# rajan-dubey8/camouflage-multimodal

Hardware: AMD Instinct MI355X
Metric: images/sec fwd+bwd (fusion model train step: fwd + loss + bwd + clip + AdamW) (higher is better)
Workload: dtype bf16; 1 GPU; BASELINE configs[1] on the path that exists (SURVEY 8d): cross-attention fusion model, packed variable-Nr minibatch (Nr ~ real 303..530 histogram, mean 483), Nk=13 real KG rows, train mode dropout 0.3, random-init weights; batch_per_gpu=16, global_batch=16, rg_dim=128, hidden_dim=256, num_heads=8, parallelism=dp1, precision=bf16 MFMA operands, fp32 accumulate/optimizer

## Files before the change

### camouflage_multimodal_amd/csrc/fused_rows.hip

```cpp
#include "fused_rows.h"
#include "shadow_inl.h"
#include "gemm.h"
#include "mfma_inl.h"

namespace {

template <int NT, int KS, bool W_IS_A, int DEPTH, bool USE_ROT = true>
struct Stage {
  static constexpr int TOTAL = NT * KS;
  static constexpr int D = DEPTH < TOTAL ? DEPTH : TOTAL;
  static_assert(!USE_ROT || (KS & (KS - 1)) == 0, "rotated k order: power-of-two k steps");
  u32x4 buf[D];
  const u32x4* wp; int rot;
  __device__ __forceinline__ int keff(int ks) const { return USE_ROT ? ((ks + rot) & (KS - 1)) : ks; }
  __device__ __forceinline__ const u32x4* wptr(int i) const { return wp + 64 * (keff(i / NT) * NT + (i % NT)); }
  __device__ __forceinline__ void prefetch(const u32x4* __restrict__ wp_, int rot_) {
    wp = wp_; rot = rot_;
#pragma unroll
    for (int i = 0; i < D; ++i) buf[i] = *wptr(i);
  }
  __device__ __forceinline__ void run(const char* act, f32x16 (&acc)[NT]) {
    run_f([&](int ks) { return *reinterpret_cast<const bf16x8*>(act + 32 * ks); }, acc);
  }
  template <class F>
// ... 967 lines not shown

constexpr int SLAB_TILES = 10;

template <int DEPTH, bool ROT>
__global__ __launch_bounds__(256, 2) void bwd2_kernel(const Bwd2Args a) {
  extern __shared__ __attribute__((aligned(16))) char smem[];
  const int tid = threadIdx.x, lane = tid & 63, l31 = lane & 31, h = lane >> 5;
  const int w = __builtin_amdgcn_readfirstlane(tid >> 6);
  const int Nk = a.Nk;
  char* Q2s = smem + X_Q2S; char* dO2s = smem + X_DO2S; float* tabs = reinterpret_cast<float*>(smem + X_TABS);
  char* bufT = smem + X_BUFT; char* imgs = smem + X_IMGS;
  int* flag = reinterpret_cast<int*>(smem + X_RED);
  const int xb = (int)blockIdx.x - a.B - a.rg_tiles_max, xearly = (a.kg_split - 1) * a.B;
  if (xb >= xearly) { ln_slab_sum(a, xb - xearly); return; }
  stamp(a.stamps, 0);
  const bool early = (int)blockIdx.x < a.B || xb >= 0;
  int b;
  if (early) {
    b = xb >= 0 ? xb % a.B : (int)blockIdx.x;
    const int kq = xb >= 0 ? 1 + xb / a.B : 0;
    const int r_lo = a.kg_split > 1 ? min(4 * kq, Nk) : 0, r_hi = a.kg_split > 1 ? min(4 * kq + 4, Nk) : Nk;
    const size_t krow0 = (size_t)b * Nk;
    Stage<2, 32, true, DEPTH, false> se;
    se.prefetch(reinterpret_cast<const u32x4*>(a.WcKgT) + (size_t)w * (48 * 2 * 64) + 64 * (16 * 2) + lane, 0);
    u32x2 du2reg[2][4];
#pragma unroll
    for (int t = 0; t < 2; ++t)
#pragma unroll
      for (int g = 0; g < 4; ++g) du2reg[t][g] = *reinterpret_cast<const u32x2*>(a.dU2_16 + (krow0 + min(l31, Nk - 1)) * 256 + 64 * w + 32 * t + 8 * g + 4 * h);
    const int t0 = a.tile_off[b], t1 = a.tile_off[b + 1];
    for (int c = tid; c < 32 * 64; c += 256) {
      const int j = c >> 6, ch = c & 63;
      u32x4 v = u32x4{0u, 0u, 0u, 0u};
      if (j >= r_lo && j < r_hi) {
        float4 x0, x1;
        if (a.slabs & 2) {
          x0 = x1 = make_float4(0.f, 0.f, 0.f, 0.f);
          const float* src = a.slabKV + (size_t)j * 512 + 8 * ch;
          for (int tb = t0; tb < t1; tb += SLAB_TILES) {
            float4 p0[SLAB_TILES], p1[SLAB_TILES];
#pragma unroll
            for (int u = 0; u < SLAB_TILES; ++u) {
              const float* s = src + (size_t)min(tb + u, t1 - 1) * Nk * 512;
              p0[u] = *reinterpret_cast<const float4*>(s); p1[u] = *reinterpret_cast<const float4*>(s + 4);
            }
#pragma unroll
            for (int u = 0; u < SLAB_TILES; ++u) {
              const bool ok = tb + u < t1;
              x0.x += ok ? p0[u].x : 0.f; x0.y += ok ? p0[u].y : 0.f; x0.z += ok ? p0[u].z : 0.f; x0.w += ok ? p0[u].w : 0.f;
              x1.x += ok ? p1[u].x : 0.f; x1.y += ok ? p1[u].y : 0.f; x1.z += ok ? p1[u].z : 0.f; x1.w += ok ? p1[u].w : 0.f;
            }
          }
          float* dst = a.dKV + (krow0 + j) * 512 + 8 * ch;
          *reinterpret_cast<float4*>(dst) = x0; *reinterpret_cast<float4*>(dst + 4) = x1;
        } else {
          const float* src = a.dKV + (krow0 + j) * 512 + 8 * ch;
          x0 = *reinterpret_cast<const float4*>(src); x1 = *reinterpret_cast<const float4*>(src + 4);
        }
        v = u32x4{pack2(x0.x, x0.y), pack2(x0.z, x0.w), pack2(x1.x, x1.y), pack2(x1.z, x1.w)};
      }
      *reinterpret_cast<u32x4*>(bufT + j * PQ + 512 + 16 * ch) = v;
    }
    __syncthreads();
    f32x16 acc[2] = {zero16(), zero16()};
    se.run(bufT + l31 * PQ + 512 + 16 * h, acc);
    copy_out<6>(bufT + r_lo * PQ, PQ, 512, a.dQKVkg16 + 256, 768, krow0 + r_lo, r_hi - r_lo);
    if (a.kg_defer) {
      us16* const dGp16 = reinterpret_cast<us16*>(a.dGpart);
      if (l31 >= r_lo && l31 < r_hi) {
#pragma unroll
        for (int t = 0; t < 2; ++t)
#pragma unroll
          for (int g = 0; g < 4; ++g) {
            const int c0 = 64 * w + 32 * t + 8 * g + 4 * h;
            const u32x2 uv = du2reg[t][g];
            *reinterpret_cast<u32x2*>(dGp16 + (krow0 + l31) * 256 + c0) =
                u32x2{pack2(acc[t][4 * g] + bf_lo(uv.x), acc[t][4 * g + 1] + bf_hi(uv.x)), pack2(acc[t][4 * g + 2] + bf_lo(uv.y), acc[t][4 * g + 3] + bf_hi(uv.y))};
          }
      }
      if (b == a.B - 1 && kq == 0) {
        const size_t tk = (size_t)a.B * Nk, n16 = (((tk + 127) & ~size_t(127)) - tk) * 32;
        for (size_t c = tid; c < n16; c += 256) *(reinterpret_cast<u32x4*>(dGp16 + tk * 256) + c) = u32x4{0u, 0u, 0u, 0u};
      }
    } else if (l31 >= r_lo && l31 < r_hi) {
#pragma unroll
      for (int t = 0; t < 2; ++t)
#pragma unroll
        for (int g = 0; g < 4; ++g) {
          const int c0 = 64 * w + 32 * t + 8 * g + 4 * h;
          const u32x2 uv = du2reg[t][g];
          float* dst = a.dGpart + (krow0 + l31) * 256 + c0;
          __hip_atomic_store(dst, acc[t][4 * g] + bf_lo(uv.x), __ATOMIC_RELAXED, __HIP_MEMORY_SCOPE_AGENT);
          __hip_atomic_store(dst + 1, acc[t][4 * g + 1] + bf_hi(uv.x), __ATOMIC_RELAXED, __HIP_MEMORY_SCOPE_AGENT);
          __hip_atomic_store(dst + 2, acc[t][4 * g + 2] + bf_lo(uv.y), __ATOMIC_RELAXED, __HIP_MEMORY_SCOPE_AGENT);
          __hip_atomic_store(dst + 3, acc[t][4 * g + 3] + bf_hi(uv.y), __ATOMIC_RELAXED, __HIP_MEMORY_SCOPE_AGENT);
        }
    }
  } else {
  const int4 td = a.tile_desc[(int)blockIdx.x - a.B];
  if (td.x < 0) return;
  b = td.x;
  const size_t rowg0 = td.y;
  const int nrows = td.z;
  const bool rok = l31 < nrows;
  const size_t vrow = rowg0 + min(l31, nrows - 1);
  Stage<2, 48, true, DEPTH, false> sr;
  sr.prefetch(reinterpret_cast<const u32x4*>(a.WcRgT) + (size_t)w * (48 * 2 * 64) + lane, 0);
// ... 451 lines not shown
  Bwd1Args k = a;
  if (kg_only) { k.rg_tiles_max = 0; k.stamps = nullptr; }
  const dim3 grid(k.B + k.rg_tiles_max + k.writer_blocks + k.nzero + k.twg.tiles);
  const double rows = (kg_only ? 0.0 : (double)a.rows_rg) + (double)a.B * a.Nk;
  const int prof = gemm_prof_open(stream, 2.0 * rows * (512.0 * 256.0 + 256.0 * 256.0) + (kg_only ? 0.0 : 10.0 * (double)a.rows_rg * a.Nk * 256.0), PROF_BWD1);
  if (variant == 0) launch_lds<bwd1_kernel<12, false>>(grid, dim3(256), W_LDS, stream, k);
  else              launch_lds<bwd1_kernel<12, true>>(grid, dim3(256), W_LDS, stream, k);
  gemm_prof_close(prof, stream);
  return (int)hipGetLastError();
}

size_t fused_bwd2_lds() { return X_LDS; }

int launch_fused_bwd2(Bwd2Args& a, int variant, hipStream_t stream) {
  (void)variant;
  if (a.B < 1 || a.Nk < 1 || a.Nk > 16 || a.rg_tiles_max < 1 || !a.Q2_16 || !a.dO2_16 || !a.lse2 || !a.delta2 || !a.KV2_16 || !a.dQKV16 ||
      !a.dU16 || !a.WcRgT || !a.dR16 || !a.dQ2acc || !a.dKV || !a.dU2_16 || !a.WcKgT || !a.dQKVkg16 || !a.dG16 || !a.dGpart || !a.tickets || !a.off || !a.tile_off || !a.tile_desc)
    return (int)hipErrorInvalidValue;
  if (!al16(a.dQKV16) || !al16(a.dQKVkg16) || !al16(a.WcRgT) || !al16(a.WcKgT) || !al16(a.dQ2acc) || !al16(a.dKV)) return (int)hipErrorInvalidValue;
  if (a.slabs && (a.param_space || (a.slabs & ~3) || !a.slabKV || !a.slabLN || !a.ln_dgamma[0] || !a.ln_dgamma[1] || !a.ln_dbeta[0] || !a.ln_dbeta[1]))
    return (int)hipErrorInvalidValue;
  if (a.param_space) a.kg_defer = 0;
  else if (a.kg_defer < 0) a.kg_defer = a.B * a.Nk <= FUSED_BWD2_DEFER_MAX_TK ? 1 : 0;
  const double dr = 2.0 * ((double)a.rows_rg * 768.0 + (double)a.B * a.Nk * (a.kg_defer ? 512.0 : 768.0)) * 256.0;
  const int prof = gemm_prof_open(stream, (a.param_space ? 0.0 : dr) + 10.0 * (double)a.rows_rg * a.Nk * 256.0, PROF_BWD2);
  if (!a.param_space) a.split_finish = 0;
  a.kg_split = (a.slabs & 2) ? 4 : 1;
  if (!a.param_space) launch_lds<bwd2_kernel<12, false>>(dim3(a.kg_split * a.B + a.rg_tiles_max + ((a.slabs & 1) ? 4 : 0)), dim3(256), X_LDS, stream, a);
  else                launch_lds<bwd2p_kernel<12, false>>(dim3(a.B + a.rg_tiles_max), dim3(256), X_LDS, stream, a);
  if (a.split_finish) hipLaunchKernelGGL(bwd2_finish_kernel, dim3(a.B), dim3(256), 0, stream, a);
  gemm_prof_close(prof, stream);
  return (int)hipGetLastError();
}
```

### camouflage_multimodal_amd/csrc/fusion_abi.hip

```cpp
#include <hip/hip_runtime.h>

#include <algorithm>
#include <cmath>
#include <cstdio>
#include <cstring>
#include <string>

#include "../../include/camo_fusion.h"

#include "attn.h"
#include "gemm.h"
#include "fused_rows.h"
#include "tail_wide.h"
#include "attn_maps.h"
#include "gemm16.h"
#include "misc.h"
#include "abi_util.h"
#include "fusion_ws.h"

namespace {
thread_local std::string g_err;
}

int camo_abi::fail(int code, const std::string& msg) { g_err = msg; return code; }
// ... 627 lines not shown
  }
  if (pl.bwd1 == CAMO_BWD1_64) CK(launch_wide2_bwd1(a1, x.opt->fused_variant, st), "fused backward, first half (64-row half-blocks)");
  else                         CK(launch_fused_bwd1(a1, x.opt->fused_variant, st), "fused backward, first half");
  if (pl.tail_event == CAMO_EVENT_AFTER_BWD1) CK(record_tail_event(c, st), "tail event");
  Bwd2Args a2; std::memset(&a2, 0, sizeof(a2));
  a2.Q2_16 = f.Q2_16; a2.dO2_16 = f.dO2_16; a2.lse2 = f.lse2; a2.delta2 = f.delta2; a2.KV2_16 = f.KV2_16; a2.dQKV16 = f.dQKV16;
  a2.dU16 = f.dU16; a2.WcRgT = sh.WcRgT; a2.dR16 = f.dR16; a2.dQ2acc = w.dQ2acc; a2.dKV = w.dKV;
  a2.slabs = a1.slabs; a2.slabKV = f.slabKV; a2.slabLN = f.slabLN;
  for (int i = 0; i < 2; ++i) { a2.ln_dgamma[i] = a1.s[i].dgamma; a2.ln_dbeta[i] = a1.s[i].dbeta; }
  a2.dU2_16 = f.dU2_16; a2.WcKgT = sh.WcKgT; a2.dQKVkg16 = f.dQKVkg16; a2.dG16 = f.dG16; a2.dGpart = f.dGpart;
  a2.tickets = w.tickets + B; a2.off = rg_offsets; a2.tile_off = bd.tile_off; a2.tile_desc = bd.tile_desc;
  a2.B = B; a2.Nk = Nk; a2.rows_rg = T; a2.rg_tiles_max = T / 32 + B; a2.qscale = a1.qscale; a2.drop = drop;
  a2.stamps = g_dbg_stamps ? g_dbg_stamps + (size_t)3 * g_dbg_stamp_blocks * 8 : nullptr;
  const bool param_space = pl.param_space != 0;
  a2.param_space = param_space ? 1 : 0;
  a2.split_finish = pl.bwd2 != CAMO_BWD2_ROWS32 ? 1 : 0;
  a2.kg_defer = x.opt->exp == 32 ? 0 : (x.opt->exp == 64 ? 1 : (x.opt->tn_big > 0 ? 0 : -1));
  if (pl.bwd2 == CAMO_BWD2_64) CK(launch_wide2_bwd2(a2, st), "fused backward, second half (64-row blocks)");
  else CK(launch_fused_bwd2(a2, x.opt->fused_variant, st), "fused backward, second half");
  if (!param_space) {
    GB16 g(drop, *x.opt, st);
    const bool kgq = a2.kg_defer == 1;
    if (kgq) {
      Gemm16Prob& p = g.tn(nullptr, H, f.KG16, D, Gr[CAMO_P_KG_PROJ_W], D, Gr[CAMO_P_KG_PROJ_B], H, D, TK);
      p.A = reinterpret_cast<const us*>(w.dQ2acc); p.flags |= GF_A_F32 | GF_KGQ;
      p.kgq_wT = sh.WcKgT; p.kgq_w = P[CAMO_P_A2_IN_W]; p.ldg = H;
      p.C16 = f.dG16; p.ldc16 = H; p.kgq_part16 = reinterpret_cast<const us*>(f.dGpart); p.kgq_a16 = f.dQKVkg16; p.kgq_lda16 = 3 * H;
    }
    g.tn(f.dH16, 2 * H, f.Y16, H, Gr[CAMO_P_F1_W0], H, Gr[CAMO_P_F1_B0], 2 * H, H, T);
    g.tn(f.dU16, H, f.O16, H, Gr[CAMO_P_A1_OUT_W], H, Gr[CAMO_P_A1_OUT_B], H, H, T);
    g.tn(f.dQKV16, 3 * H, f.R16, H, Gr[CAMO_P_A1_IN_W], H, Gr[CAMO_P_A1_IN_B], H, H, T);
    g.tn(f.dQKV16 + H, 3 * H, f.R16, H, Gr[CAMO_P_A2_IN_W] + HH, H, Gr[CAMO_P_A2_IN_B] + H, 2 * H, H, T);
    g.tn(f.dR16, H, f.X16, D, Gr[CAMO_P_RG_PROJ_W], D, Gr[CAMO_P_RG_PROJ_B], H, D, T);
    g.tn(f.dH2_16, 2 * H, f.Y2_16, H, Gr[CAMO_P_F2_W0], H, Gr[CAMO_P_F2_B0], 2 * H, H, TK);
    g.tn(f.dU2_16, H, f.O2_16, H, Gr[CAMO_P_A2_OUT_W], H, Gr[CAMO_P_A2_OUT_B], H, H, TK);
    if (kgq) {
      Gemm16Prob& p = g.tn(nullptr, H, f.G16, H, Gr[CAMO_P_A2_IN_W], H, Gr[CAMO_P_A2_IN_B], H, H, TK);
      p.A = reinterpret_cast<const us*>(w.dQ2acc); p.flags |= GF_A_F32;
    } else {
      g.tn(f.dQKVkg16, 3 * H, f.G16, H, Gr[CAMO_P_A2_IN_W], H, Gr[CAMO_P_A2_IN_B], H, H, TK);
    }
    g.tn(f.dQKVkg16 + H, 3 * H, f.G16, H, Gr[CAMO_P_A1_IN_W] + HH, H, Gr[CAMO_P_A1_IN_B] + H, 2 * H, H, TK);
    g.tn(kgq ? reinterpret_cast<const us*>(f.dGpart) : f.dG16, H, f.KG16, D, Gr[CAMO_P_KG_PROJ_W], D, Gr[CAMO_P_KG_PROJ_B], H, D, TK);
    CK(g.run(), "node-level weight gradients");
    return 0;
  }
  float* const Mrg = w.parM.Mrg; float* const Mkg = w.parM.Mkg; float* const dbrg = w.parM.dbrg; float* const dbkg = w.parM.dbkg;
  GB16 g(drop, *x.opt, st);
  g.tn(f.dH16, 2 * H, f.Y16, H, Gr[CAMO_P_F1_W0], H, Gr[CAMO_P_F1_B0], 2 * H, H, T);
  g.tn(f.dU16, H, f.O16, H, Gr[CAMO_P_A1_OUT_W], H, Gr[CAMO_P_A1_OUT_B], H, H, T);
  g.tn(f.dQKV16, 3 * H, f.X16, D, Mrg, D, dbrg, H, D, T).bias_grad2 = Gr[CAMO_P_A1_IN_B];
  g.tn(f.dQKV16 + H, 3 * H, f.X16, D, Mrg + (size_t)H * D, D, dbrg + H, 2 * H, D, T).bias_grad2 = Gr[CAMO_P_A2_IN_B] + H;
  g.tn(f.dU16, H, f.X16, D, Gr[CAMO_P_RG_PROJ_W], D, Gr[CAMO_P_RG_PROJ_B], H, D, T);
  g.tn(f.dH2_16, 2 * H, f.Y2_16, H, Gr[CAMO_P_F2_W0], H, Gr[CAMO_P_F2_B0], 2 * H, H, TK);
  g.tn(f.dU2_16, H, f.O2_16, H, Gr[CAMO_P_A2_OUT_W], H, Gr[CAMO_P_A2_OUT_B], H, H, TK);
  g.tn(f.dQKVkg16, 3 * H, f.KG16, D, Mkg, D, dbkg, H, D, TK).bias_grad2 = Gr[CAMO_P_A2_IN_B];
  g.tn(f.dQKVkg16 + H, 3 * H, f.KG16, D, Mkg + (size_t)H * D, D, dbkg + H, 2 * H, D, TK).bias_grad2 = Gr[CAMO_P_A1_IN_B] + H;
  g.tn(f.dU2_16, H, f.KG16, D, Gr[CAMO_P_KG_PROJ_W], D, Gr[CAMO_P_KG_PROJ_B], H, D, TK);
  CK(g.run(), "node-level weight gradients");
  {
    const UnfoldStream urg{Mrg, dbrg, P[CAMO_P_A1_IN_W], P[CAMO_P_A2_IN_W] + HH, P[CAMO_P_RG_PROJ_W], P[CAMO_P_RG_PROJ_B], Gr[CAMO_P_A1_IN_W],
                           Gr[CAMO_P_A2_IN_W] + HH, Gr[CAMO_P_RG_PROJ_W], Gr[CAMO_P_RG_PROJ_B]};
    const UnfoldStream ukg{Mkg, dbkg, P[CAMO_P_A2_IN_W], P[CAMO_P_A1_IN_W] + HH, P[CAMO_P_KG_PROJ_W], P[CAMO_P_KG_PROJ_B], Gr[CAMO_P_A2_IN_W],
                           Gr[CAMO_P_A1_IN_W] + HH, Gr[CAMO_P_KG_PROJ_W], Gr[CAMO_P_KG_PROJ_B]};
    CK(launch_unfold(urg, ukg, st), "projection / in-projection weight gradients (parameter space)");
  }
// ... 475 lines not shown
```

### camouflage_multimodal_amd/csrc/gemm16.h

```cpp
#pragma once
#include "common.h"
#include "gemm.h"

#define GEMM16_MAXP 12

struct Gemm16Prob {
  const unsigned short* A; const unsigned short* B;
  float* C;
  unsigned short* C16;
  const float* bias;
  const float* res;
  float* bias_grad;
  float* bias_grad2;
  int M, N, K;
  int lda, ldb, ldc, ldc16, ldr;
  int flags;
  uint32_t drop_site;
  float aux_scale;
  const int* row_sample; const float* inv_nr; int uniform_n;
  float* colmean; int ldm;
  int ln_mode;
  const float* ln_gamma; const float* ln_beta; float* ln_stats; const float* ln_x; float* ln_dgamma; float* ln_dbeta;
  const float* virt_g; int ldg;
  const unsigned short* kgq_wT; const float* kgq_w;
  const unsigned short* kgq_part16; unsigned short* kgq_a16; int kgq_lda16;
  int tiles_n, ksplit, kchunk, tile_begin;
};

struct Gemm16Batch {
  Gemm16Prob p[GEMM16_MAXP];
  int n;
  DropCfg drop;
  int exp;
  int n_heavy;
};

struct Gemm16Knobs {
  int tn_big = -1;
  int balance = 1;
  int tn_kcap = 0;
  int exp = 0;
};

int launch_gemm16_batch(Gemm16Batch& gb, const Gemm16Knobs& kn, hipStream_t stream);
```

### camouflage_multimodal_amd/csrc/gemm16.hip

```cpp
#include "gemm16.h"
#include "mfma_inl.h"
#include <type_traits>


namespace {

constexpr int BM = 64, BN = 128, BK = 64;
constexpr int PM = 128;
constexpr int PKA = 192, PKB = 320;
constexpr int A_NT_BYTES = BM * PM;
constexpr int A_TN_BYTES = BK * PKA;
constexpr int NT_BUF_BYTES = (BM + BN) * PM;
constexpr int BUF_BYTES = 32768;

struct Stage { u32x4 a[2], b[4]; };
struct StageF { float4 a[4]; u32x4 b[4]; int ok; };

__device__ __forceinline__ u32x4 virt_chunk(u32x4 act, float4 g0, float4 g1, float scale) {
  auto sel = [&](uint32_t bits, float g) { return __uint_as_float(bits) > 0.f ? g * scale : 0.f; };
  u32x4 o;
  o.x = pack2(sel(act.x << 16, g0.x), sel(act.x & 0xFFFF0000u, g0.y));
  o.y = pack2(sel(act.y << 16, g0.z), sel(act.y & 0xFFFF0000u, g0.w));
  o.z = pack2(sel(act.z << 16, g1.x), sel(act.z & 0xFFFF0000u, g1.y));
  o.w = pack2(sel(act.w << 16, g1.z), sel(act.w & 0xFFFF0000u, g1.w));
// ... 144 lines not shown
    const int s_first = srow[0];
    const bool one = srow[63] == s_first || (srow[63] < 0 && srow[min(M - 1 - m0, 63)] == s_first);
    float sum = 0.f; int cur = -1;
    for (int r = 0; r < 32; ++r) {
      const int sm = srow[half * 32 + r];
      if (sm < 0) break;
      if (sm != cur) {
        if (cur >= 0 && col < N) atomicAdd(P.colmean + (size_t)cur * P.ldm + col, sum * (P.row_sample ? P.inv_nr[cur] : 1.0f / (float)P.uniform_n));
        sum = 0.f; cur = sm;
      }
      sum += tile[(half * 32 + r) * TP + t];
    }
    if (one) {
      if (half == 1) hsum[t] = sum;
      __syncthreads();
      if (half == 0 && col < N && cur >= 0)
        atomicAdd(P.colmean + (size_t)cur * P.ldm + col, (sum + hsum[t]) * (P.row_sample ? P.inv_nr[cur] : 1.0f / (float)P.uniform_n));
    } else if (cur >= 0 && col < N) {
      atomicAdd(P.colmean + (size_t)cur * P.ldm + col, sum * (P.row_sample ? P.inv_nr[cur] : 1.0f / (float)P.uniform_n));
    }
  }
}

__device__ __forceinline__ void kgq_finish(const Gemm16Prob& P, int m0, int q, const f32x16 (&acc)[2], const f32x16& accb, char* smem) {
  const int tid = threadIdx.x, lane = tid & 63, wave = tid >> 6;
  const int wr = wave >> 1, wc = wave & 1, l31 = lane & 31, h = lane >> 5;
  constexpr int PT = 144;
  const u32x4* wp = reinterpret_cast<const u32x4*>(P.kgq_wT) + ((size_t)(q * 48 + (m0 >> 4)) * 2 + wr) * 64 + lane;
  u32x4 wf[4];
#pragma unroll
  for (int s = 0; s < 4; ++s) wf[s] = wp[128 * s];
  float* sv = reinterpret_cast<float*>(smem + 128 * PT);
#pragma unroll
  for (int j = 0; j < 2; ++j) {
    char* row = smem + (64 * wc + 32 * j + l31) * PT + 2 * (32 * wr + 4 * h);
#pragma unroll
    for (int g = 0; g < 4; ++g)
      *reinterpret_cast<u32x2*>(row + 16 * g) = u32x2{pack2(acc[j][4 * g], acc[j][4 * g + 1]), pack2(acc[j][4 * g + 2], acc[j][4 * g + 3])};
  }
  if (wc == 0 && l31 == 0) {
#pragma unroll
    for (int r = 0; r < 16; ++r) sv[32 * wr + acc_row(r, h)] = accb[r];
  }
  __syncthreads();
  f32x16 o[2] = {zero16(), zero16()};
#pragma unroll
  for (int s = 0; s < 4; ++s) {
    const char* pb = smem + (64 * wc + l31) * PT + 32 * s + 16 * h;
    const bf16x8 b0 = *reinterpret_cast<const bf16x8*>(pb), b1 = *reinterpret_cast<const bf16x8*>(pb + 32 * PT);
    o[0] = __builtin_amdgcn_mfma_f32_32x32x16_bf16(as_frag(wf[s]), b0, o[0], 0, 0, 0);
    o[1] = __builtin_amdgcn_mfma_f32_32x32x16_bf16(as_frag(wf[s]), b1, o[1], 0, 0, 0);
  }
#pragma unroll
  for (int j = 0; j < 2; ++j) {
    float* cp = P.C + 64 * wc + 32 * j + l31;
#pragma unroll
    for (int r = 0; r < 16; ++r) atomicAdd(cp + (size_t)(64 * q + 32 * wr + acc_row(r, h)) * P.ldc, o[j][r]);
  }
  {
    const int i = tid & 63, j0 = 16 * (tid >> 6);
    const float* w = P.kgq_w + (size_t)(m0 + j0) * P.ldg + 64 * q + i;
    float sum = 0.f;
#pragma unroll
    for (int j = 0; j < 16; ++j) sum = fmaf(w[(size_t)j * P.ldg], sv[j0 + j], sum);
    atomicAdd(P.bias_grad + 64 * q + i, sum);
  }
}

__device__ __forceinline__ void kgq_rows(const Gemm16Prob& P, int r0, char* smem) {
  const int tid = threadIdx.x, lane = tid & 63, w = tid >> 6, l31 = lane & 31, h = lane >> 5;
  constexpr int PR_ = 528;
  for (int c = tid; c < 32 * 32; c += 256) {
    const int j = c >> 5, ch = c & 31, row = r0 + j;
    u32x4 v = u32x4{0u, 0u, 0u, 0u};
    if (row < P.K) {
      const float* src = reinterpret_cast<const float*>(P.A) + (size_t)row * P.lda + 8 * ch;
      const float4 x0 = *reinterpret_cast<const float4*>(src), x1 = *reinterpret_cast<const float4*>(src + 4);
      v = u32x4{pack2(x0.x, x0.y), pack2(x0.z, x0.w), pack2(x1.x, x1.y), pack2(x1.z, x1.w)};
      *reinterpret_cast<u32x4*>(P.kgq_a16 + (size_t)row * P.kgq_lda16 + 8 * ch) = v;
    }
    *reinterpret_cast<u32x4*>(smem + j * PR_ + 16 * ch) = v;
  }
  __syncthreads();
  const u32x4* wp = reinterpret_cast<const u32x4*>(P.kgq_wT) + (size_t)w * (48 * 2 * 64) + lane;
  f32x16 acc[2] = {zero16(), zero16()};
#pragma unroll 4
  for (int ks = 0; ks < 16; ++ks) {
    const bf16x8 x = *reinterpret_cast<const bf16x8*>(smem + l31 * PR_ + 32 * ks + 16 * h);
    acc[0] = __builtin_amdgcn_mfma_f32_32x32x16_bf16(as_frag(wp[64 * (2 * ks)]), x, acc[0], 0, 0, 0);
    acc[1] = __builtin_amdgcn_mfma_f32_32x32x16_bf16(as_frag(wp[64 * (2 * ks + 1)]), x, acc[1], 0, 0, 0);
  }
  const int row = r0 + l31;
  if (row < P.K) {
#pragma unroll
    for (int t = 0; t < 2; ++t)
#pragma unroll
      for (int g = 0; g < 4; ++g) {
        const int c0 = 64 * w + 32 * t + 8 * g + 4 * h;
        const u32x2 pv = *reinterpret_cast<const u32x2*>(P.kgq_part16 + (size_t)row * P.ldc16 + c0);
        *reinterpret_cast<u32x2*>(P.C16 + (size_t)row * P.ldc16 + c0) =
            u32x2{pack2(acc[t][4 * g] + bf_lo(pv.x), acc[t][4 * g + 1] + bf_hi(pv.x)), pack2(acc[t][4 * g + 2] + bf_lo(pv.y), acc[t][4 * g + 3] + bf_hi(pv.y))};
      }
  }
}

template <int PIPE, bool VIRT, bool F32A = false>
__device__ __forceinline__ void body_tn(const Gemm16Prob& P, int m0, int n0, int kt0, int nt, char* smem, int exp = 0, int rq = 0) {
  const int tid = threadIdx.x, lane = tid & 63, wave = tid >> 6;
  const int wr = wave >> 1, wc = wave & 1, l31 = lane & 31, h = lane >> 5;
  const int M = P.M, N = P.N;

  uint32_t goa[2], gob[4];
  int la[2], lb[4];
#pragma unroll
  for (int i = 0; i < 2; ++i) {
    const int s = tid + 256 * i, kr = s >> 3, c = s & 7;
    goa[i] = ((uint32_t)kr * (uint32_t)P.lda + (uint32_t)min(m0 + 8 * c, M - 8)) * 2u;
    la[i] = kr * PKA + 16 * c;
  }
#pragma unroll
  for (int i = 0; i < 4; ++i) {
    const int s = tid + 256 * i, kr = s >> 4, c = s & 15;
    gob[i] = ((uint32_t)kr * (uint32_t)P.ldb + (uint32_t)min(n0 + 8 * c, N - 8)) * 2u;
    lb[i] = A_TN_BYTES + kr * PKB + 16 * c;
  }
  const char* Ab = reinterpret_cast<const char*>(P.A);
  const char* Bb = reinterpret_cast<const char*>(P.B);
  const size_t astep = (size_t)BK * P.lda * 2, bstep = (size_t)BK * P.ldb * 2;

  f32x16 acc[2], accb;
// ... 3 lines not shown
  const short one = (short)0x3F80;
  const bf16x8 ones = {one, one, one, one, one, one, one, one};
  std::conditional_t<F32A, StageF, Stage> st[PIPE];
  int sa[PIPE][2];
  float* gs = reinterpret_cast<float*>(smem + 2 * BUF_BYTES);
  if constexpr (VIRT) {
    const int ns = P.uniform_n > 0 && !P.row_sample ? (P.K + P.uniform_n - 1) / P.uniform_n : P.ldc16;
    for (int i = tid; i < ns * 64; i += 256) {
      const int sm = i >> 6, f = i & 63, c = min(m0 + f, M - 1);
      const float inv = P.row_sample ? P.inv_nr[sm] : 1.0f / (float)P.uniform_n;
      gs[i] = P.virt_g[(size_t)sm * P.ldg + c] * inv * P.aux_scale;
    }
    __syncthreads();
  }

  auto gload = [&](auto& r, int (&srow)[2], int kt) {
    const int k = kt0 + min(kt, nt - 1);
    const char* a = Ab + (size_t)k * astep;
    const char* b = Bb + (size_t)k * bstep;
    if constexpr (F32A) {
      r.ok = 0;
#pragma unroll
      for (int i = 0; i < 2; ++i) {
        const int s = tid + 256 * i, row = k * BK + (s >> 3);
        const float* src = reinterpret_cast<const float*>(P.A) + (size_t)min(row, P.K - 1) * P.lda + min(m0 + 8 * (s & 7), M - 8);
        r.a[2 * i] = *reinterpret_cast<const float4*>(src); r.a[2 * i + 1] = *reinterpret_cast<const float4*>(src + 4);
        r.ok |= row < P.K ? 1 << i : 0;
      }
    } else {
#pragma unroll
      for (int i = 0; i < 2; ++i) r.a[i] = *reinterpret_cast<const u32x4*>(a + goa[i]);
    }
#pragma unroll
    for (int i = 0; i < 4; ++i) r.b[i] = *reinterpret_cast<const u32x4*>(b + gob[i]);
    if constexpr (VIRT) {
#pragma unroll
      for (int i = 0; i < 2; ++i) {
        const int node = min(k * BK + ((tid + 256 * i) >> 3), P.K - 1);
        srow[i] = P.row_sample ? P.row_sample[node] : node / P.uniform_n;
      }
    }
  };
  auto sstore = [&](const auto& r, const int (&srow)[2], int buf) {
    char* base = smem + buf * BUF_BYTES;
#pragma unroll
    for (int i = 0; i < 2; ++i) {
      u32x4 a;
      if constexpr (F32A) {
// ... 14 lines not shown
  };
  const int g = (lane >> 4) & 1, q = (lane >> 2) & 3, p = lane & 3;
  const int fa = (8 * h + q) * PKA + 64 * wr + 32 * g + 8 * p;
  const int fb = A_TN_BYTES + (8 * h + q) * PKB + 128 * wc + 32 * g + 8 * p;
  auto compute = [&](int buf) {
    const char* base = smem + buf * BUF_BYTES;
#pragma unroll
    for (int s = 0; s < 4; ++s) {
      const char* pa = base + fa + 16 * s * PKA;
      const char* pb = base + fb + 16 * s * PKB;
      const s16x4 a0 = lds_tr16(pa), a1 = lds_tr16(pa + 4 * PKA);
      const s16x4 b00 = lds_tr16(pb), b01 = lds_tr16(pb + 4 * PKB);
      const s16x4 b10 = lds_tr16(pb + 64), b11 = lds_tr16(pb + 64 + 4 * PKB);
      const bf16x8 a = {a0.x, a0.y, a0.z, a0.w, a1.x, a1.y, a1.z, a1.w};
      const bf16x8 b0 = {b00.x, b00.y, b00.z, b00.w, b01.x, b01.y, b01.z, b01.w};
      const bf16x8 b1 = {b10.x, b10.y, b10.z, b10.w, b11.x, b11.y, b11.z, b11.w};
      acc[0] = __builtin_amdgcn_mfma_f32_32x32x16_bf16(a, b0, acc[0], 0, 0, 0);
      acc[1] = __builtin_amdgcn_mfma_f32_32x32x16_bf16(a, b1, acc[1], 0, 0, 0);
      if (do_bsum) accb = __builtin_amdgcn_mfma_f32_32x32x16_bf16(a, ones, accb, 0, 0, 0);
    }
  };
  auto gloadi = [&](int j, int kt) { gload(st[j], sa[j], kt); };
  auto sstorei = [&](int j, int buf) { sstore(st[j], sa[j], buf); };
  G16_PIPELINE_LOOP

  if constexpr (F32A) {
    if (P.flags & GF_KGQ) { kgq_finish(P, m0, rq, acc, accb, smem); return; }
  }
  const int rowb = m0 + wr * 32 + 4 * h;
  if ((exp & 1) && acc[0][0] != 12345.f) return;
  if (do_bsum && l31 == 0) {
#pragma unroll
    for (int r = 0; r < 16; ++r) {
      const int row = rowb + (r & 3) + 8 * (r >> 2);
      if (row < M) { atomicAdd(P.bias_grad + row, accb[r]); if (P.bias_grad2) atomicAdd(P.bias_grad2 + row, accb[r]); }
    }
  }
#pragma unroll
  for (int j = 0; j < 2; ++j) {
    const int col = n0 + wc * 64 + j * 32 + l31;
    if (col >= N) continue;
    float* cp = P.C + col;
#pragma unroll
    for (int r = 0; r < 16; ++r) {
      const int row = rowb + (r & 3) + 8 * (r >> 2);
      if (row < M) atomicAdd(cp + (size_t)row * P.ldc, acc[j][r]);
    }
  }
}


// ... 176 lines not shown
    const float m1 = row_total(s1, 0) * invN;
    const float m2 = row_total(s2, 1) * invN;
#pragma unroll
    for (int j = 0; j < 2; ++j)
#pragma unroll
      for (int g = 0; g < 4; ++g) {
        const int c0 = w * 64 + j * 32 + 8 * g + 4 * h;
        float4 du;
        du.x = (gq[j][g].x - m1 - xq[j][g].x * m2) * rstd; du.y = (gq[j][g].y - m1 - xq[j][g].y * m2) * rstd;
        du.z = (gq[j][g].z - m1 - xq[j][g].z * m2) * rstd; du.w = (gq[j][g].w - m1 - xq[j][g].w * m2) * rstd;
        if (rok) {
          if (P.C) *reinterpret_cast<float4*>(P.C + (size_t)row * P.ldc + c0) = du;
          if (P.C16) *reinterpret_cast<uint2*>(P.C16 + (size_t)row * P.ldc16 + c0) = make_uint2(pack2(du.x, du.y), pack2(du.z, du.w));
        }
      }
    const int nrow = min(RM, M - m0);
    float a = 0.f, b = 0.f;
    for (int r = 0; r < nrow; ++r) { a += tile0[r * TPR + tid]; b += tile1[r * TPR + tid]; }
    atomicAdd(P.ln_dgamma + tid, a);
    atomicAdd(P.ln_dbeta + tid, b);
  }
}

template <int PIPE, bool ROWS>
__global__ __launch_bounds__(256, ROWS ? 2 : 3) void gemm16_kernel(const Gemm16Batch gb, int total_tiles) {
  extern __shared__ __attribute__((aligned(16))) char smem_raw[];
  int bid = blockIdx.x;
  {
    const int nwg = total_tiles, q = nwg >> 3, r = nwg & 7, xcd = bid & 7, j = bid >> 3;
    const int first = xcd * q + min(xcd, r);
    if (gb.n_heavy > 0) {
      const int nh = gb.n_heavy, qh = nh >> 3, rh = nh & 7;
      const int hc = qh + (xcd < rh ? 1 : 0), hfirst = xcd * qh + min(xcd, rh);
      bid = j < hc ? hfirst + j : nh + (first - hfirst) + (j - hc);
    } else {
      bid = first + j;
    }
  }
  int pi = 0;
#pragma unroll
  for (int i = 1; i < GEMM16_MAXP; ++i)
    if (i < gb.n && bid >= gb.p[i].tile_begin) pi = i;
  const Gemm16Prob& P = gb.p[pi];
  int t = bid - P.tile_begin;
  if constexpr (ROWS) {
    if (P.ln_mode) {
      if (P.flags & GF_A_VIRT) body_nt_row<PIPE, true>(gb, P, t * RM, smem_raw);
      else                     body_nt_row<PIPE, false>(gb, P, t * RM, smem_raw);
      return;
    }
  }
  const int tiles = ((P.M + BM - 1) / BM) * P.tiles_n;
  if ((P.flags & GF_KGQ) && t >= tiles * P.ksplit) { kgq_rows(P, (t - tiles * P.ksplit) * 32, smem_raw); return; }
  const int ks = t / tiles; t -= ks * tiles;
  const int tn = t % P.tiles_n, tm = t / P.tiles_n;
  if (P.flags & GF_A_KMAJOR) {
    const int ktiles = (P.K + 127) / 128 * 2;
    const int per = P.kchunk / BK, kt0 = ks * per;
    if (P.flags & GF_A_F32) {
      if (P.flags & GF_KGQ) body_tn<PIPE, false, true>(P, tm * BM, 0, 0, ktiles, smem_raw, 0, ks);
      else                  body_tn<PIPE, false, true>(P, tm * BM, tn * BN, kt0, min(per, ktiles - kt0), smem_raw);
      return;
    }
    if constexpr (ROWS) {
      if (P.flags & GF_A_VIRT) { body_tn<PIPE, true>(P, tm * BM, tn * BN, kt0, min(per, ktiles - kt0), smem_raw); return; }
    }
    body_tn<PIPE, false>(P, tm * BM, tn * BN, kt0, (gb.exp & 2) ? 2 : min(per, ktiles - kt0), smem_raw, gb.exp);
  } else {
    body_nt<PIPE>(gb, P, tm * BM, tn * BN, smem_raw);
  }
}

constexpr int GM = 128, GN = 256;
constexpr int GPA = 320, GPB = 576;
constexpr int GA_BYTES = BK * GPA;
constexpr int GBUF_BYTES = GA_BYTES + BK * GPB;

template <int PIPE>
__global__ __launch_bounds__(512) void gemm16_tnbig_kernel(const Gemm16Batch gb, int total_tiles) {
  extern __shared__ __attribute__((aligned(16))) char smem[];
  int bid = blockIdx.x;
  {
    const int nwg = total_tiles, q = nwg >> 3, r = nwg & 7, xcd = bid & 7, j = bid >> 3;
// ... 164 lines not shown
    int extra = 0;
    for (int i = 0; i < gb.n; ++i) {
      Gemm16Prob& p = gb.p[i];
      const bool akm = p.flags & GF_A_KMAJOR, bkm = p.flags & GF_B_KMAJOR;
      if (akm != bkm || p.M < 1 || p.N < 1 || p.K < 1) return (int)hipErrorInvalidValue;
      if (!al16(p.A) || !al16(p.B) || (p.lda & 7) || (p.ldb & 7)) return (int)hipErrorInvalidValue;
      if ((double)(akm ? p.K + 128 : p.M) * p.lda * 2.0 >= 4.0e9 || (double)(akm ? p.K + 128 : p.N) * p.ldb * 2.0 >= 4.0e9)
        return (int)hipErrorInvalidValue;
      p.tiles_n = (p.N + BN - 1) / BN;
      int tiles = ((p.M + BM - 1) / BM) * p.tiles_n;
      if (p.ln_mode) {
        if (akm || p.N != RN || !p.ln_gamma || !al16(p.ln_gamma) || (p.ln_mode == 1 && (!p.ln_beta || !al16(p.ln_beta))) ||
            (p.ln_mode == 2 && (!p.ln_x || !al16(p.ln_x) || !p.ln_stats || !p.ln_dgamma || !p.ln_dbeta)) ||
            (p.flags & (GF_RELU | GF_DROPOUT | GF_RELU_BWD)))
          return (int)hipErrorInvalidValue;
        p.tiles_n = 1;
        tiles = (p.M + RM - 1) / RM;
      }
      if (akm) {
        if ((p.M & 7) || (p.N & 7) || p.M < 8 || p.N < 8 || !p.C || (p.C16 && !(p.flags & GF_KGQ)) || p.bias || p.res ||
            (p.flags & ~(GF_A_KMAJOR | GF_B_KMAJOR | GF_ATOMIC | GF_A_VIRT | GF_A_F32 | GF_KGQ)))
          return (int)hipErrorInvalidValue;
        if ((p.flags & GF_A_F32) && ((p.flags & GF_A_VIRT) || (double)p.K * p.lda * 4.0 >= 4.0e9)) return (int)hipErrorInvalidValue;
        if ((p.flags & GF_KGQ) && (!(p.flags & GF_A_F32) || p.M != 256 || p.N != BN || !p.kgq_wT || !al16(p.kgq_wT) || !p.kgq_w || p.ldg < 256 || !p.bias_grad ||
                                   !p.C16 || !p.kgq_part16 || !p.kgq_a16 || (reinterpret_cast<uintptr_t>(p.C16) & 7) || (reinterpret_cast<uintptr_t>(p.kgq_part16) & 7) ||
                                   !al16(p.kgq_a16) || p.ldc16 < 256 || (p.ldc16 & 3) || p.kgq_lda16 < 256 || (p.kgq_lda16 & 7)))
          return (int)hipErrorInvalidValue;
        if (p.flags & GF_A_VIRT) {
          const int ns = p.row_sample ? p.ldc16 : (p.uniform_n > 0 ? (p.K + p.uniform_n - 1) / p.uniform_n : 0);
          if (!p.virt_g || ns < 1 || ns * 256 > 2 * ROW_BUF_BYTES - 2 * BUF_BYTES || (!p.row_sample && p.uniform_n < 1))
            return (int)hipErrorInvalidValue;
        }
        const int ktiles = (p.K + 127) / 128 * 2;
        const int per = ktiles < kcap ? ktiles : kcap;
        p.kchunk = per * BK;
        p.ksplit = (ktiles + per - 1) / per;
        if (p.flags & GF_KGQ) { p.kchunk = ktiles * BK; p.ksplit = 4; extra += tiles * 4 + (p.K + 31) / 32; }
      } else {
        if ((p.K % BK) || (p.N & 3) || (p.flags & (GF_ATOMIC | GF_SIGMOID)) || p.bias_grad) return (int)hipErrorInvalidValue;
        if ((p.C && (!al16(p.C) || (p.ldc & 3))) || (p.C16 && ((reinterpret_cast<uintptr_t>(p.C16) & 7) || (p.ldc16 & 3))) ||
            (p.bias && !al16(p.bias)) || (p.res && (!al16(p.res) || (p.ldr & 3))) || (p.colmean && !p.row_sample && p.uniform_n < 1))
          return (int)hipErrorInvalidValue;
        p.kchunk = p.K; p.ksplit = 1;
      }
      p.tile_begin = total;
      total += tiles * p.ksplit + ((p.flags & GF_KGQ) ? (p.K + 31) / 32 : 0);
    }
    if (kn.tn_kcap > 0 || (kcap > 16 ? total - extra >= 440 : total - extra >= 200) || kcap <= KCAP_MIN) break;
  }
  gb.n_heavy = 0; gb.exp = kn.exp;
  if (kn.balance && kcap_used <= 16) {
    int i = 0;
    while (i < gb.n && (gb.p[i].flags & GF_A_KMAJOR) && gb.p[i].ksplit > 1) ++i;
    const int first_light = i;
    while (i < gb.n && (gb.p[i].flags & GF_A_KMAJOR) && gb.p[i].ksplit == 1) ++i;
    if (i == gb.n && first_light > 0 && first_light < gb.n) gb.n_heavy = gb.p[first_light].tile_begin;
  }
  bool has_tn = false, has_rows = false, has_virt = false;
  for (int i = 0; i < gb.n; ++i) {
    has_tn = has_tn || (gb.p[i].flags & GF_A_KMAJOR); has_rows = has_rows || gb.p[i].ln_mode;
    has_virt = has_virt || (gb.p[i].flags & GF_A_VIRT);
    if ((gb.p[i].flags & GF_A_VIRT) && !(gb.p[i].flags & GF_A_KMAJOR) && (!gb.p[i].ln_mode || !gb.p[i].virt_g || (gb.p[i].ldg & 3)))
      return (int)hipErrorInvalidValue;
  }
  if (has_virt && !has_rows) return (int)hipErrorInvalidValue;
  double fl = 0.0;
  for (int i = 0; i < gb.n; ++i) {
    const Gemm16Prob& p = gb.p[i];
    if (p.flags & GF_KGQ) fl += 2.0 * p.M * (double)p.N * (4.0 * p.K + 256.0) + 2.0 * p.K * 256.0 * 256.0;
    else fl += 2.0 * p.M * (double)p.N * p.K;
  }
  const int prof = gemm_prof_open(stream, fl);
  if (!has_rows && !has_tn) hipLaunchKernelGGL((gemm16_kernel<2, false>), dim3(total), dim3(256), 2 * NT_BUF_BYTES, stream, gb, total);
  else if (!has_rows)       launch_lds<gemm16_kernel<2, false>>(dim3(total), dim3(256), 2 * BUF_BYTES, stream, gb, total);
  else                      launch_lds<gemm16_kernel<2, true>>(dim3(total), dim3(256), 2 * ROW_BUF_BYTES, stream, gb, total);
  gemm_prof_close(prof, stream);
  return (int)hipGetLastError();
}
```

Before: 104,000 images/s.

## Move deferred KG dG GEMM from bwd2 into the KGQ weight-gradient batch

When kg_defer is set, the bwd2 kernel no longer runs the KG-row MFMA against WcKgT or writes the bf16 dG partial. Instead the KGQ problem in the weight-gradient GEMM batch now spans three 256-wide M slices, including the dKV part. Each block loops over the slices, accumulating the bias-gradient and output contributions before one set of atomics. kgq_rows now reads all 768 input columns. This removes a GEMM and a round trip through memory from the latency-critical bwd2 kernel. In exchange the batched kernel does more per-block serial work, and the TN-only launch now uses a template variant capped at 2 blocks per CU.

```diff
diff --git a/camouflage_multimodal_amd/csrc/fused_rows.hip b/camouflage_multimodal_amd/csrc/fused_rows.hip
--- a/camouflage_multimodal_amd/csrc/fused_rows.hip
+++ b/camouflage_multimodal_amd/csrc/fused_rows.hip
@@ -1013,12 +1013,14 @@
     const int r_lo = a.kg_split > 1 ? min(4 * kq, Nk) : 0, r_hi = a.kg_split > 1 ? min(4 * kq + 4, Nk) : Nk;
     const size_t krow0 = (size_t)b * Nk;
     Stage<2, 32, true, DEPTH, false> se;
-    se.prefetch(reinterpret_cast<const u32x4*>(a.WcKgT) + (size_t)w * (48 * 2 * 64) + 64 * (16 * 2) + lane, 0);
-    u32x2 du2reg[2][4];
-#pragma unroll
-    for (int t = 0; t < 2; ++t)
-#pragma unroll
-      for (int g = 0; g < 4; ++g) du2reg[t][g] = *reinterpret_cast<const u32x2*>(a.dU2_16 + (krow0 + min(l31, Nk - 1)) * 256 + 64 * w + 32 * t + 8 * g + 4 * h);
+    u32x2 du2reg[2][4] = {};
+    if (!a.kg_defer) {
+      se.prefetch(reinterpret_cast<const u32x4*>(a.WcKgT) + (size_t)w * (48 * 2 * 64) + 64 * (16 * 2) + lane, 0);
+#pragma unroll
+      for (int t = 0; t < 2; ++t)
+#pragma unroll
+        for (int g = 0; g < 4; ++g) du2reg[t][g] = *reinterpret_cast<const u32x2*>(a.dU2_16 + (krow0 + min(l31, Nk - 1)) * 256 + 64 * w + 32 * t + 8 * g + 4 * h);
+    }
     const int t0 = a.tile_off[b], t1 = a.tile_off[b + 1];
     for (int c = tid; c < 32 * 64; c += 256) {
       const int j = c >> 6, ch = c & 63;
@@ -1054,26 +1056,9 @@
     }
     __syncthreads();
     f32x16 acc[2] = {zero16(), zero16()};
-    se.run(bufT + l31 * PQ + 512 + 16 * h, acc);
+    if (!a.kg_defer) se.run(bufT + l31 * PQ + 512 + 16 * h, acc);
     copy_out<6>(bufT + r_lo * PQ, PQ, 512, a.dQKVkg16 + 256, 768, krow0 + r_lo, r_hi - r_lo);
-    if (a.kg_defer) {
-      us16* const dGp16 = reinterpret_cast<us16*>(a.dGpart);
-      if (l31 >= r_lo && l31 < r_hi) {
-#pragma unroll
-        for (int t = 0; t < 2; ++t)
-#pragma unroll
-          for (int g = 0; g < 4; ++g) {
-            const int c0 = 64 * w + 32 * t + 8 * g + 4 * h;
-            const u32x2 uv = du2reg[t][g];
-            *reinterpret_cast<u32x2*>(dGp16 + (krow0 + l31) * 256 + c0) =
-                u32x2{pack2(acc[t][4 * g] + bf_lo(uv.x), acc[t][4 * g + 1] + bf_hi(uv.x)), pack2(acc[t][4 * g + 2] + bf_lo(uv.y), acc[t][4 * g + 3] + bf_hi(uv.y))};
-          }
-      }
-      if (b == a.B - 1 && kq == 0) {
-        const size_t tk = (size_t)a.B * Nk, n16 = (((tk + 127) & ~size_t(127)) - tk) * 32;
-        for (size_t c = tid; c < n16; c += 256) *(reinterpret_cast<u32x4*>(dGp16 + tk * 256) + c) = u32x4{0u, 0u, 0u, 0u};
-      }
-    } else if (l31 >= r_lo && l31 < r_hi) {
+    if (!a.kg_defer && l31 >= r_lo && l31 < r_hi) {
 #pragma unroll
       for (int t = 0; t < 2; ++t)
 #pragma unroll
@@ -1571,7 +1556,7 @@
     return (int)hipErrorInvalidValue;
   if (a.param_space) a.kg_defer = 0;
   else if (a.kg_defer < 0) a.kg_defer = a.B * a.Nk <= FUSED_BWD2_DEFER_MAX_TK ? 1 : 0;
-  const double dr = 2.0 * ((double)a.rows_rg * 768.0 + (double)a.B * a.Nk * (a.kg_defer ? 512.0 : 768.0)) * 256.0;
+  const double dr = 2.0 * ((double)a.rows_rg * 768.0 + (double)a.B * a.Nk * (a.kg_defer ? 0.0 : 768.0)) * 256.0;
   const int prof = gemm_prof_open(stream, (a.param_space ? 0.0 : dr) + 10.0 * (double)a.rows_rg * a.Nk * 256.0, PROF_BWD2);
   if (!a.param_space) a.split_finish = 0;
   a.kg_split = (a.slabs & 2) ? 4 : 1;
diff --git a/camouflage_multimodal_amd/csrc/fusion_abi.hip b/camouflage_multimodal_amd/csrc/fusion_abi.hip
--- a/camouflage_multimodal_amd/csrc/fusion_abi.hip
+++ b/camouflage_multimodal_amd/csrc/fusion_abi.hip
@@ -673,10 +673,11 @@
     GB16 g(drop, *x.opt, st);
     const bool kgq = a2.kg_defer == 1;
     if (kgq) {
-      Gemm16Prob& p = g.tn(nullptr, H, f.KG16, D, Gr[CAMO_P_KG_PROJ_W], D, Gr[CAMO_P_KG_PROJ_B], H, D, TK);
+      Gemm16Prob& p = g.tn(nullptr, H, f.KG16, D, Gr[CAMO_P_KG_PROJ_W], D, Gr[CAMO_P_KG_PROJ_B], 3 * H, D, TK);
       p.A = reinterpret_cast<const us*>(w.dQ2acc); p.flags |= GF_A_F32 | GF_KGQ;
-      p.kgq_wT = sh.WcKgT; p.kgq_w = P[CAMO_P_A2_IN_W]; p.ldg = H;
-      p.C16 = f.dG16; p.ldc16 = H; p.kgq_part16 = reinterpret_cast<const us*>(f.dGpart); p.kgq_a16 = f.dQKVkg16; p.kgq_lda16 = 3 * H;
+      p.kgq_A2 = w.dKV; p.kgq_lda2 = 2 * H;
+      p.kgq_wT = sh.WcKgT; p.kgq_w = P[CAMO_P_A2_IN_W]; p.kgq_w2 = P[CAMO_P_A1_IN_W] + HH; p.ldg = H;
+      p.C16 = f.dG16; p.ldc16 = H; p.kgq_part16 = f.dU2_16; p.kgq_a16 = f.dQKVkg16; p.kgq_lda16 = 3 * H;
     }
     g.tn(f.dH16, 2 * H, f.Y16, H, Gr[CAMO_P_F1_W0], H, Gr[CAMO_P_F1_B0], 2 * H, H, T);
     g.tn(f.dU16, H, f.O16, H, Gr[CAMO_P_A1_OUT_W], H, Gr[CAMO_P_A1_OUT_B], H, H, T);
@@ -692,7 +693,7 @@
       g.tn(f.dQKVkg16, 3 * H, f.G16, H, Gr[CAMO_P_A2_IN_W], H, Gr[CAMO_P_A2_IN_B], H, H, TK);
     }
     g.tn(f.dQKVkg16 + H, 3 * H, f.G16, H, Gr[CAMO_P_A1_IN_W] + HH, H, Gr[CAMO_P_A1_IN_B] + H, 2 * H, H, TK);
-    g.tn(kgq ? reinterpret_cast<const us*>(f.dGpart) : f.dG16, H, f.KG16, D, Gr[CAMO_P_KG_PROJ_W], D, Gr[CAMO_P_KG_PROJ_B], H, D, TK);
+    g.tn(kgq ? f.dU2_16 : f.dG16, H, f.KG16, D, Gr[CAMO_P_KG_PROJ_W], D, Gr[CAMO_P_KG_PROJ_B], H, D, TK);
     CK(g.run(), "node-level weight gradients");
     return 0;
   }
diff --git a/camouflage_multimodal_amd/csrc/gemm16.h b/camouflage_multimodal_amd/csrc/gemm16.h
--- a/camouflage_multimodal_amd/csrc/gemm16.h
+++ b/camouflage_multimodal_amd/csrc/gemm16.h
@@ -22,7 +22,8 @@
   int ln_mode;
   const float* ln_gamma; const float* ln_beta; float* ln_stats; const float* ln_x; float* ln_dgamma; float* ln_dbeta;
   const float* virt_g; int ldg;
-  const unsigned short* kgq_wT; const float* kgq_w;
+  const unsigned short* kgq_wT; const float* kgq_w; const float* kgq_w2;
+  const float* kgq_A2; int kgq_lda2;
   const unsigned short* kgq_part16; unsigned short* kgq_a16; int kgq_lda16;
   int tiles_n, ksplit, kchunk, tile_begin;
 };
diff --git a/camouflage_multimodal_amd/csrc/gemm16.hip b/camouflage_multimodal_amd/csrc/gemm16.hip
--- a/camouflage_multimodal_amd/csrc/gemm16.hip
+++ b/camouflage_multimodal_amd/csrc/gemm16.hip
@@ -190,7 +190,8 @@
   }
 }
 
-__device__ __forceinline__ void kgq_finish(const Gemm16Prob& P, int m0, int q, const f32x16 (&acc)[2], const f32x16& accb, char* smem) {
+__device__ __forceinline__ void kgq_slice(const Gemm16Prob& P, int m0, int q, const f32x16 (&acc)[2], const f32x16& accb, char* smem,
+                                          f32x16 (&o)[2], float& bsum) {
   const int tid = threadIdx.x, lane = tid & 63, wave = tid >> 6;
   const int wr = wave >> 1, wc = wave & 1, l31 = lane & 31, h = lane >> 5;
   constexpr int PT = 144;
@@ -211,7 +212,6 @@
     for (int r = 0; r < 16; ++r) sv[32 * wr + acc_row(r, h)] = accb[r];
   }
   __syncthreads();
-  f32x16 o[2] = {zero16(), zero16()};
 #pragma unroll
   for (int s = 0; s < 4; ++s) {
     const char* pb = smem + (64 * wc + l31) * PT + 32 * s + 16 * h;
@@ -219,33 +219,39 @@
     o[0] = __builtin_amdgcn_mfma_f32_32x32x16_bf16(as_frag(wf[s]), b0, o[0], 0, 0, 0);
     o[1] = __builtin_amdgcn_mfma_f32_32x32x16_bf16(as_frag(wf[s]), b1, o[1], 0, 0, 0);
   }
+  {
+    const int i = tid & 63, j0 = 16 * (tid >> 6);
+    const float* w = (m0 < 256 ? P.kgq_w + (size_t)(m0 + j0) * P.ldg : P.kgq_w2 + (size_t)(m0 - 256 + j0) * P.ldg) + 64 * q + i;
+#pragma unroll
+    for (int j = 0; j < 16; ++j) bsum = fmaf(w[(size_t)j * P.ldg], sv[j0 + j], bsum);
+  }
+  __syncthreads();
+}
+
+__device__ __forceinline__ void kgq_store(const Gemm16Prob& P, int q, const f32x16 (&o)[2], float bsum) {
+  const int tid = threadIdx.x, lane = tid & 63, wave = tid >> 6;
+  const int wr = wave >> 1, wc = wave & 1, l31 = lane & 31, h = lane >> 5;
 #pragma unroll
   for (int j = 0; j < 2; ++j) {
     float* cp = P.C + 64 * wc + 32 * j + l31;
 #pragma unroll
     for (int r = 0; r < 16; ++r) atomicAdd(cp + (size_t)(64 * q + 32 * wr + acc_row(r, h)) * P.ldc, o[j][r]);
   }
-  {
-    const int i = tid & 63, j0 = 16 * (tid >> 6);
-    const float* w = P.kgq_w + (size_t)(m0 + j0) * P.ldg + 64 * q + i;
-    float sum = 0.f;
-#pragma unroll
-    for (int j = 0; j < 16; ++j) sum = fmaf(w[(size_t)j * P.ldg], sv[j0 + j], sum);
-    atomicAdd(P.bias_grad + 64 * q + i, sum);
-  }
+  atomicAdd(P.bias_grad + 64 * q + (tid & 63), bsum);
 }
 
 __device__ __forceinline__ void kgq_rows(const Gemm16Prob& P, int r0, char* smem) {
   const int tid = threadIdx.x, lane = tid & 63, w = tid >> 6, l31 = lane & 31, h = lane >> 5;
-  constexpr int PR_ = 528;
-  for (int c = tid; c < 32 * 32; c += 256) {
-    const int j = c >> 5, ch = c & 31, row = r0 + j;
+  constexpr int PR_ = 1552;
+  for (int c = tid; c < 32 * 96; c += 256) {
+    const int j = c / 96, ch = c - 96 * j, row = r0 + j;
     u32x4 v = u32x4{0u, 0u, 0u, 0u};
     if (row < P.K) {
-      const float* src = reinterpret_cast<const float*>(P.A) + (size_t)row * P.lda + 8 * ch;
+      const float* src = ch < 32 ? reinterpret_cast<const float*>(P.A) + (size_t)row * P.lda + 8 * ch
+                                 : P.kgq_A2 + (size_t)row * P.kgq_lda2 + 8 * (ch - 32);
       const float4 x0 = *reinterpret_cast<const float4*>(src), x1 = *reinterpret_cast<const float4*>(src + 4);
       v = u32x4{pack2(x0.x, x0.y), pack2(x0.z, x0.w), pack2(x1.x, x1.y), pack2(x1.z, x1.w)};
-      *reinterpret_cast<u32x4*>(P.kgq_a16 + (size_t)row * P.kgq_lda16 + 8 * ch) = v;
+      if (ch < 32) *reinterpret_cast<u32x4*>(P.kgq_a16 + (size_t)row * P.kgq_lda16 + 8 * ch) = v;
     }
     *reinterpret_cast<u32x4*>(smem + j * PR_ + 16 * ch) = v;
   }
@@ -253,7 +259,7 @@
   const u32x4* wp = reinterpret_cast<const u32x4*>(P.kgq_wT) + (size_t)w * (48 * 2 * 64) + lane;
   f32x16 acc[2] = {zero16(), zero16()};
 #pragma unroll 4
-  for (int ks = 0; ks < 16; ++ks) {
+  for (int ks = 0; ks < 48; ++ks) {
     const bf16x8 x = *reinterpret_cast<const bf16x8*>(smem + l31 * PR_ + 32 * ks + 16 * h);
     acc[0] = __builtin_amdgcn_mfma_f32_32x32x16_bf16(as_frag(wp[64 * (2 * ks)]), x, acc[0], 0, 0, 0);
     acc[1] = __builtin_amdgcn_mfma_f32_32x32x16_bf16(as_frag(wp[64 * (2 * ks + 1)]), x, acc[1], 0, 0, 0);
@@ -273,7 +279,7 @@
 }
 
 template <int PIPE, bool VIRT, bool F32A = false>
-__device__ __forceinline__ void body_tn(const Gemm16Prob& P, int m0, int n0, int kt0, int nt, char* smem, int exp = 0, int rq = 0) {
+__device__ __forceinline__ void body_tn(const Gemm16Prob& P, int m0, int n0, int kt0, int nt, char* smem, int exp = 0, int rq = 0, int mstep = 0) {
   const int tid = threadIdx.x, lane = tid & 63, wave = tid >> 6;
   const int wr = wave >> 1, wc = wave & 1, l31 = lane & 31, h = lane >> 5;
   const int M = P.M, N = P.N;
@@ -323,8 +329,9 @@
       r.ok = 0;
 #pragma unroll
       for (int i = 0; i < 2; ++i) {
-        const int s = tid + 256 * i, row = k * BK + (s >> 3);
-        const float* src = reinterpret_cast<const float*>(P.A) + (size_t)min(row, P.K - 1) * P.lda + min(m0 + 8 * (s & 7), M - 8);
+        const int s = tid + 256 * i, row = k * BK + (s >> 3), col = min(m0 + 8 * (s & 7), M - 8);
+        const float* src = (P.flags & GF_KGQ) && m0 >= 256 ? P.kgq_A2 + (size_t)min(row, P.K - 1) * P.kgq_lda2 + (col - 256)
+                                                           : reinterpret_cast<const float*>(P.A) + (size_t)min(row, P.K - 1) * P.lda + col;
         r.a[2 * i] = *reinterpret_cast<const float4*>(src); r.a[2 * i + 1] = *reinterpret_cast<const float4*>(src + 4);
         r.ok |= row < P.K ? 1 << i : 0;
       }
@@ -385,11 +392,24 @@
   };
   auto gloadi = [&](int j, int kt) { gload(st[j], sa[j], kt); };
   auto sstorei = [&](int j, int buf) { sstore(st[j], sa[j], buf); };
+  if constexpr (F32A) {
+    if (P.flags & GF_KGQ) {
+      f32x16 o[2] = {zero16(), zero16()};
+      float bsum = 0.f;
+      for (;;) {
+        G16_PIPELINE_LOOP
+        kgq_slice(P, m0, rq, acc, accb, smem, o, bsum);
+        m0 += mstep;
+        if (mstep <= 0 || m0 >= M) break;
+#pragma unroll
+        for (int r = 0; r < 16; ++r) { acc[0][r] = 0.f; acc[1][r] = 0.f; accb[r] = 0.f; }
+      }
+      kgq_store(P, rq, o, bsum);
+      return;
+    }
+  }
   G16_PIPELINE_LOOP
 
-  if constexpr (F32A) {
-    if (P.flags & GF_KGQ) { kgq_finish(P, m0, rq, acc, accb, smem); return; }
-  }
   const int rowb = m0 + wr * 32 + 4 * h;
   if ((exp & 1) && acc[0][0] != 12345.f) return;
   if (do_bsum && l31 == 0) {
@@ -612,8 +632,8 @@
   }
 }
 
-template <int PIPE, bool ROWS>
-__global__ __launch_bounds__(256, ROWS ? 2 : 3) void gemm16_kernel(const Gemm16Batch gb, int total_tiles) {
+template <int PIPE, bool ROWS, bool TN = false>
+__global__ __launch_bounds__(256, ROWS || TN ? 2 : 3) void gemm16_kernel(const Gemm16Batch gb, int total_tiles) {
   extern __shared__ __attribute__((aligned(16))) char smem_raw[];
   int bid = blockIdx.x;
   {
@@ -640,15 +660,17 @@
       return;
     }
   }
-  const int tiles = ((P.M + BM - 1) / BM) * P.tiles_n;
-  if ((P.flags & GF_KGQ) && t >= tiles * P.ksplit) { kgq_rows(P, (t - tiles * P.ksplit) * 32, smem_raw); return; }
+  const int tiles = (P.flags & GF_KGQ) ? (P.M / BM) / 3 : ((P.M + BM - 1) / BM) * P.tiles_n;
+  if constexpr (ROWS || TN) {
+    if ((P.flags & GF_KGQ) && t >= tiles * P.ksplit) { kgq_rows(P, (t - tiles * P.ksplit) * 32, smem_raw); return; }
+  }
   const int ks = t / tiles; t -= ks * tiles;
   const int tn = t % P.tiles_n, tm = t / P.tiles_n;
   if (P.flags & GF_A_KMAJOR) {
     const int ktiles = (P.K + 127) / 128 * 2;
     const int per = P.kchunk / BK, kt0 = ks * per;
-    if (P.flags & GF_A_F32) {
-      if (P.flags & GF_KGQ) body_tn<PIPE, false, true>(P, tm * BM, 0, 0, ktiles, smem_raw, 0, ks);
+    if constexpr (ROWS || TN) if (P.flags & GF_A_F32) {
+      if (P.flags & GF_KGQ) body_tn<PIPE, false, true>(P, tm * BM, 0, 0, (P.K + BK - 1) / BK, smem_raw, 0, ks, tiles * BM);
       else                  body_tn<PIPE, false, true>(P, tm * BM, tn * BN, kt0, min(per, ktiles - kt0), smem_raw);
       return;
     }
@@ -859,7 +881,8 @@
             (p.flags & ~(GF_A_KMAJOR | GF_B_KMAJOR | GF_ATOMIC | GF_A_VIRT | GF_A_F32 | GF_KGQ)))
           return (int)hipErrorInvalidValue;
         if ((p.flags & GF_A_F32) && ((p.flags & GF_A_VIRT) || (double)p.K * p.lda * 4.0 >= 4.0e9)) return (int)hipErrorInvalidValue;
-        if ((p.flags & GF_KGQ) && (!(p.flags & GF_A_F32) || p.M != 256 || p.N != BN || !p.kgq_wT || !al16(p.kgq_wT) || !p.kgq_w || p.ldg < 256 || !p.bias_grad ||
+        if ((p.flags & GF_KGQ) && (!(p.flags & GF_A_F32) || p.M != 768 || p.N != BN || !p.kgq_wT || !al16(p.kgq_wT) || !p.kgq_w || !p.kgq_w2 || p.ldg < 256 || !p.bias_grad ||
+                                   p.lda < 256 || (p.lda & 3) || !p.kgq_A2 || !al16(p.kgq_A2) || p.kgq_lda2 < 512 || (p.kgq_lda2 & 3) || (double)p.K * p.kgq_lda2 * 4.0 >= 4.0e9 ||
                                    !p.C16 || !p.kgq_part16 || !p.kgq_a16 || (reinterpret_cast<uintptr_t>(p.C16) & 7) || (reinterpret_cast<uintptr_t>(p.kgq_part16) & 7) ||
                                    !al16(p.kgq_a16) || p.ldc16 < 256 || (p.ldc16 & 3) || p.kgq_lda16 < 256 || (p.kgq_lda16 & 7)))
           return (int)hipErrorInvalidValue;
@@ -872,7 +895,10 @@
         const int per = ktiles < kcap ? ktiles : kcap;
         p.kchunk = per * BK;
         p.ksplit = (ktiles + per - 1) / per;
-        if (p.flags & GF_KGQ) { p.kchunk = ktiles * BK; p.ksplit = 4; extra += tiles * 4 + (p.K + 31) / 32; }
+        if (p.flags & GF_KGQ) {
+          tiles /= 3;
+          p.kchunk = ktiles * BK; p.ksplit = 4; extra += tiles * 4 + (p.K + 31) / 32;
+        }
       } else {
         if ((p.K % BK) || (p.N & 3) || (p.flags & (GF_ATOMIC | GF_SIGMOID)) || p.bias_grad) return (int)hipErrorInvalidValue;
         if ((p.C && (!al16(p.C) || (p.ldc & 3))) || (p.C16 && ((reinterpret_cast<uintptr_t>(p.C16) & 7) || (p.ldc16 & 3))) ||
@@ -904,12 +930,12 @@
   double fl = 0.0;
   for (int i = 0; i < gb.n; ++i) {
     const Gemm16Prob& p = gb.p[i];
-    if (p.flags & GF_KGQ) fl += 2.0 * p.M * (double)p.N * (4.0 * p.K + 256.0) + 2.0 * p.K * 256.0 * 256.0;
+    if (p.flags & GF_KGQ) fl += 2.0 * p.M * (double)p.N * (4.0 * p.K + 256.0) + 2.0 * p.K * (double)p.M * 256.0;
     else fl += 2.0 * p.M * (double)p.N * p.K;
   }
   const int prof = gemm_prof_open(stream, fl);
   if (!has_rows && !has_tn) hipLaunchKernelGGL((gemm16_kernel<2, false>), dim3(total), dim3(256), 2 * NT_BUF_BYTES, stream, gb, total);
-  else if (!has_rows)       launch_lds<gemm16_kernel<2, false>>(dim3(total), dim3(256), 2 * BUF_BYTES, stream, gb, total);
+  else if (!has_rows)       launch_lds<gemm16_kernel<2, false, true>>(dim3(total), dim3(256), 2 * BUF_BYTES, stream, gb, total);
   else                      launch_lds<gemm16_kernel<2, true>>(dim3(total), dim3(256), 2 * ROW_BUF_BYTES, stream, gb, total);
   gemm_prof_close(prof, stream);
   return (int)hipGetLastError();
```

Measured after the change: 104,600 images/s (median of 6 runs). Within noise of the previous version (+0.5%).
